# Iamctb/ImageStitching

Hardware: AMD Instinct MI355X
Metric: stitched megapixels/sec (9x12 MP vertical) (higher is better)
Workload: dtype u8

## Files before the change

imagestitching_amd/csrc/ist_ctx.h:

```cpp
#ifndef IST_CTX_H_
#define IST_CTX_H_

#include <hip/hip_runtime_api.h>

#include <memory>
#include <mutex>
#include <vector>

#include "ist_jpeg.h"

#include "ist_host.h"
#include "ist_internal.h"
#include "ist_launch.h"

struct ist_ctx {
  int device = 0;
  hipStream_t stream = nullptr;
  void* scratch_src = nullptr; size_t scratch_src_bytes = 0;
  void* scratch_dst = nullptr; size_t scratch_dst_bytes = 0;
  void* scratch_dec = nullptr; size_t scratch_dec_bytes = 0;
  void* scratch_huff = nullptr; size_t scratch_huff_bytes = 0;
  void* scratch_png = nullptr; size_t scratch_png_bytes = 0;
  void* scratch_file = nullptr; size_t scratch_file_bytes = 0;
  void* scratch_jpg = nullptr; size_t scratch_jpg_bytes = 0;
  void* scratch_arena = nullptr; size_t scratch_arena_bytes = 0;
  std::vector<hipStream_t> img_stream;
  std::vector<hipEvent_t> img_event;
  std::vector<void*> img_huff; std::vector<size_t> img_huff_bytes;
  std::unique_ptr<ist::WorkerPool> workers;
  std::vector<ist::ScanBuf> scan_bufs;
  std::vector<ist::ScanBuf> file_bufs;
  void* scratch_ent = nullptr; size_t scratch_ent_bytes = 0;
  hipStream_t render = nullptr;
  hipEvent_t render_done = nullptr;
  hipStream_t png2 = nullptr;
  hipStream_t aux = nullptr;
  static constexpr int kTablePool = 32;
  struct TableBlock { uint8_t* p; size_t bytes; };
  std::vector<TableBlock> table_pool;
  std::mutex table_mu;
  std::mutex mu;
  int png_level = 1;
  std::unique_ptr<ist::Stager> stager;
  bool timing_on = false;
  double last_ms[IST_PHASE_COUNT] = {0, 0, 0, 0, 0, 0, 0, 0};
  static constexpr int kBatchRing = 4;
  struct BatchSlot { void* host = nullptr; void* dev = nullptr; size_t bytes = 0; hipEvent_t done = nullptr; bool pending = false; };
  BatchSlot batch_ring[kBatchRing];
  int batch_next = 0;
  std::mutex batch_mu;
  struct BatchHalf {
    void* tab = nullptr; size_t tab_bytes = 0;
    void* src = nullptr; size_t src_bytes = 0;
    void* dst = nullptr; size_t dst_bytes = 0;
    void* file = nullptr; size_t file_bytes = 0;
    hipEvent_t kernel_done = nullptr;
    hipEvent_t read_done = nullptr;
  };
  BatchHalf batch_half[2];
  void* scratch_prev = nullptr; size_t scratch_prev_bytes = 0;
  hipEvent_t prev_done = nullptr; bool prev_pending = false; hipStream_t prev_last = nullptr;
  ist_job* prev_job = nullptr;
  int64_t prev_job_key[5] = {0, 0, 0, 0, 0};
  std::mutex prev_mu;
  void* prev_out = nullptr; size_t prev_out_bytes = 0;
  hipStream_t prev_stream = nullptr;
  hipEvent_t prev_ready = nullptr;
};

namespace ist {
struct DevTables {
  DevOp* ops = nullptr;
  DevCell* cells = nullptr;
  DevBand* bands = nullptr;
  int32_t* stacks = nullptr;
  DevTile* tiles = nullptr;
};
}

struct ist_job {
  ist_ctx* ctx = nullptr;
  ist::Compiled host;
  std::unique_ptr<ist::FlatTwin> flat;
  ist::DevTables flat_dt;
  uint8_t* d_tables = nullptr;
  size_t d_tables_bytes = 0;
  static constexpr int kStreams = 4;
  hipStream_t launched_on[kStreams] = {nullptr, nullptr, nullptr, nullptr};
  int n_launched_on = 0;
  bool launched = false, launched_many = false;
  std::mutex launch_mu;
  ist::DevTables dt;
  int max_image = -1;
};

#define IST_HIP(expr) do { const hipError_t e_ = (expr); if (e_ != hipSuccess) return ist::fail(IST_E_HIP, std::string(#expr) + ": " + hipGetErrorString(e_)); } while (0)
#define IST_HIP_OR(expr, msg) do { if ((expr) != hipSuccess) { (void)hipGetLastError(); return ist::fail(IST_E_HIP, msg); } } while (0)

namespace ist {

struct DeviceGuard {
  int prev = -1;
  bool ok = false;
  explicit DeviceGuard(int dev) {
    if (hipGetDevice(&prev) != hipSuccess) prev = -1;
    ok = hipSetDevice(dev) == hipSuccess;
  }
  ~DeviceGuard() { if (prev >= 0) (void)hipSetDevice(prev); }
};

int grow_device(void** p, size_t* have, size_t need);
inline size_t arena_take(size_t* off, size_t bytes) { const size_t at = *off; *off += round256(bytes); return at; }

ist_job* job_compile(ist_ctx* ctx, int64_t canvas_w, int64_t canvas_h, const uint8_t clear_rgba[4], const ist_op* ops, int n_ops,
                     const ist_image_desc* images, int n_images, int filter, const ist_region* clip);
struct TableLayout { size_t bytes[2][5] = {}; size_t at[2][5] = {}; const void* from[2][5] = {}; size_t total = 0; };
TableLayout table_layout(const ist_job& job);
void pack_tables(const TableLayout& L, uint8_t* blob);
void point_tables(ist_job* job, const TableLayout& L, uint8_t* base);
int job_launch_args(const ist_job* job, const void* const* src, const size_t* src_pitch, int n_images, void* dst, size_t dst_pitch,
                    LaunchArgs* out, const Compiled** out_run, bool* out_flat);
void note_launch_stream(ist_job* job, void* stream);
void count_flat_launches(int64_t n);

int batch_take_slot(ist_ctx* ctx, size_t bytes, ist_ctx::BatchSlot** out);

inline Stager& stager_of(ist_ctx* ctx) { if (!ctx->stager) ctx->stager.reset(new Stager(ctx->device)); return *ctx->stager; }
inline WorkerPool& workers_of(ist_ctx* ctx) { if (!ctx->workers) ctx->workers.reset(new WorkerPool()); return *ctx->workers; }
int ensure_aux(ist_ctx* ctx);
int ensure_render(ist_ctx* ctx);
int read_back_pooled(const void* dev, size_t bytes, hipStream_t stream, uint8_t** out);
int png_to_host(ist_ctx* ctx, const void* canvas, size_t pitch, int64_t w, int64_t h, void* dfile, uint8_t** out_png, int64_t* out_len,
                const std::function<int(int64_t, void*)>& need_rows = nullptr, int64_t slab_rows_hint = 0, ist_preview* preview = nullptr);

int jpeg_to_host(ist_ctx* ctx, const void* canvas, size_t pitch, int64_t w, int64_t h, int quality, int subsampling, uint8_t** out_jpeg,
                 int64_t* out_len);
int jpeg_check_options(const char* who, int quality, int subsampling);
int jpeg_check_export(const char* who, int64_t w, int64_t h, int quality, int subsampling);

int preview_check(ist_preview* pv);
inline void preview_clear(ist_preview* pv) { if (pv) { pv->width = pv->height = 0; pv->pixels = nullptr; } }
int preview_enqueue(ist_ctx* ctx, const void* src, size_t src_pitch, int64_t w, int64_t h, bool opaque, void* dst, size_t dst_pitch,
                    int32_t pw, int32_t ph, hipStream_t stream);
int preview_event(ist_ctx* ctx);
void bitmap_view(const ist_bitmap* b, int* device, const uint8_t** row0, size_t* pitch, ist_image_desc* desc);
struct PreviewTail {
  ist_ctx* ctx; const void* canvas; size_t pitch; int64_t w, h; ist_preview* pv;
  int32_t pw = 0, ph = 0;
  uint8_t* host = nullptr;
  bool queued = false;
  PreviewTail(ist_ctx* c, const void* cv, size_t p, int64_t w_, int64_t h_, ist_preview* v) : ctx(c), canvas(cv), pitch(p), w(w_), h(h_), pv(v) {}
  ~PreviewTail();
  int prepare();
  int queue(hipStream_t reader);
  int finish();
};

}

#endif
```

imagestitching_amd/csrc/ist_host.cpp:

```cpp
#include "ist_host.h"

#include <algorithm>
#include <atomic>
#include <cstring>
#include <mutex>
#include <string>
#include <thread>

#include "ist_internal.h"

namespace ist {

namespace {

constexpr size_t kPoolGranule = 2u << 20;
constexpr size_t kPoolKeepBytes = 2ull << 30;
constexpr size_t kPoolKeepBlocks = 6;

constexpr size_t kPoolKeepBatchBytes = 8ull << 30;
constexpr size_t kPoolKeepBatchBlocks = 256;

struct Block { void* p; size_t cap; bool busy; uint64_t stamp; bool batch = false; };
std::mutex g_pool_mu;
std::vector<Block>& pool() { static std::vector<Block>* v = new std::vector<Block>(); return *v; }
uint64_t g_pool_clock = 0;

void pool_enforce_class_locked(bool batch) {
  const size_t keep_bytes = batch ? kPoolKeepBatchBytes : kPoolKeepBytes, keep_blocks = batch ? kPoolKeepBatchBlocks : kPoolKeepBlocks;
  for (;;) {
    size_t idle_bytes = 0, idle = 0, oldest = SIZE_MAX;
    std::vector<Block>& v = pool();
    for (size_t i = 0; i < v.size(); ++i) {
      if (v[i].busy || v[i].batch != batch) continue;
      idle_bytes += v[i].cap; ++idle;
      if (oldest == SIZE_MAX || v[i].stamp < v[oldest].stamp) oldest = i;
    }
    if (oldest == SIZE_MAX || (idle_bytes <= keep_bytes && idle <= keep_blocks)) return;
    (void)hipHostFree(v[oldest].p);
    v.erase(v.begin() + static_cast<std::ptrdiff_t>(oldest));
  }
}

void* pool_take_class(size_t bytes, bool batch) {
  const size_t need = ((bytes ? bytes : 1) + kPoolGranule - 1) / kPoolGranule * kPoolGranule;
  {
    std::lock_guard<std::mutex> lock(g_pool_mu);
    std::vector<Block>& v = pool();
    size_t best = SIZE_MAX;
    for (size_t i = 0; i < v.size(); ++i)
      if (!v[i].busy && v[i].batch == batch && v[i].cap >= need && v[i].cap <= 2 * need && (best == SIZE_MAX || v[i].cap < v[best].cap)) best = i;
    if (best != SIZE_MAX) { v[best].busy = true; v[best].stamp = ++g_pool_clock; return v[best].p; }
  }
  void* p = nullptr;
  if (hipHostMalloc(&p, need, hipHostMallocPortable) != hipSuccess) {
    (void)hipGetLastError();
    pool_trim();
    if (hipHostMalloc(&p, need, hipHostMallocPortable) != hipSuccess) { (void)hipGetLastError(); return nullptr; }
  }
  std::lock_guard<std::mutex> lock(g_pool_mu);
  pool().push_back(Block{p, need, true, ++g_pool_clock, batch});
  return p;
}
// ... 53 lines not shown
  uint8_t* d = static_cast<uint8_t*>(it.host_dst) + p.row0 * it.host_pitch + p.col0;
  if (it.host_pitch == p.n_cols) { std::memcpy(d, chunk, p.n_rows * p.n_cols); return; }
  for (size_t r = 0; r < p.n_rows; ++r) std::memcpy(d + r * it.host_pitch, chunk + r * p.n_cols, p.n_cols);
}
inline uint8_t* dev_of(const RowsCopy& it, const Piece& p) { return static_cast<uint8_t*>(it.dev) + p.row0 * it.row + p.col0; }

}

void Stager::release_lane(Lane& l) {
  if (l.stream) (void)hipStreamSynchronize(l.stream);
  for (int s = 0; s < 2; ++s) { if (l.done[s]) (void)hipEventDestroy(l.done[s]); if (l.chunk[s]) (void)hipHostFree(l.chunk[s]); l.done[s] = nullptr; l.chunk[s] = nullptr; }
  if (l.tail) (void)hipEventDestroy(l.tail);
  if (l.stream) (void)hipStreamDestroy(l.stream);
  l.tail = nullptr; l.stream = nullptr;
}

Stager::~Stager() {
  int prev = -1;
  (void)hipGetDevice(&prev);
  if (hipSetDevice(device_) != hipSuccess) return;
  if (big_.stream) (void)hipStreamSynchronize(big_.stream);
  for (int s = 0; s < 2; ++s) { if (big_.done[s]) (void)hipEventDestroy(big_.done[s]); if (big_.piece[s]) (void)hipHostFree(big_.piece[s]); }
  if (big_.tail) (void)hipEventDestroy(big_.tail);
  if (big_.stream) (void)hipStreamDestroy(big_.stream);
  for (Lane& l : lanes_) release_lane(l);
  if (gate_) (void)hipEventDestroy(gate_);
  if (prev >= 0) (void)hipSetDevice(prev);
}

int Stager::ensure() {
  if (!lanes_.empty()) return IST_OK;
  std::vector<Lane> lanes(kLanes);
  hipEvent_t gate = nullptr;
  bool ok = hipEventCreateWithFlags(&gate, hipEventDisableTiming) == hipSuccess;
  for (Lane& l : lanes) {
    ok = ok && hipStreamCreateWithFlags(&l.stream, hipStreamNonBlocking) == hipSuccess &&
         hipEventCreateWithFlags(&l.tail, hipEventDisableTiming) == hipSuccess;
    for (int s = 0; s < 2 && ok; ++s)
      ok = hipHostMalloc(&l.chunk[s], kChunk, hipHostMallocDefault) == hipSuccess &&
           hipEventCreateWithFlags(&l.done[s], hipEventDisableTiming) == hipSuccess &&
           hipEventRecord(l.done[s], l.stream) == hipSuccess;
  }
  if (!ok) {
    (void)hipGetLastError();
    for (Lane& l : lanes) release_lane(l);
    if (gate) (void)hipEventDestroy(gate);
    return fail(IST_E_HIP, "allocating the pinned staging ring failed");
  }
  lanes_.swap(lanes);
  gate_ = gate;
  return IST_OK;
}

namespace { constexpr size_t kBigPiece = 32u << 20; constexpr int kBigPackers = 4; }

int Stager::ensure_big() {
  if (big_.stream) return IST_OK;
  Big b;
  bool ok = hipStreamCreateWithFlags(&b.stream, hipStreamNonBlocking) == hipSuccess && hipEventCreateWithFlags(&b.tail, hipEventDisableTiming) == hipSuccess;
  for (int s = 0; s < 2 && ok; ++s)
    ok = hipHostMalloc(&b.piece[s], kBigPiece, hipHostMallocDefault) == hipSuccess && hipEventCreateWithFlags(&b.done[s], hipEventDisableTiming) == hipSuccess &&
         hipEventRecord(b.done[s], b.stream) == hipSuccess;
  if (!ok) {
    (void)hipGetLastError();
    for (int s = 0; s < 2; ++s) { if (b.done[s]) (void)hipEventDestroy(b.done[s]); if (b.piece[s]) (void)hipHostFree(b.piece[s]); }
    if (b.tail) (void)hipEventDestroy(b.tail);
    if (b.stream) (void)hipStreamDestroy(b.stream);
    return fail(IST_E_HIP, "allocating the large staging pieces failed");
  }
  big_ = b;
  return IST_OK;
}

int Stager::upload_big(const std::vector<RowsCopy>& items, hipStream_t after, WorkerPool* pool) {
  if (!pool) return upload(items, after);
  std::vector<RowsCopy> small;
  bool any = false;
  for (const RowsCopy& it : items) { if (it.row == 0 || it.rows == 0) continue; if (it.row > kBigPiece) small.push_back(it); else any = true; }
  if (!small.empty()) { const int rc = upload(small, after); if (rc) return rc; }
  if (!any) return IST_OK;
  int rc = ensure_big();
  if (rc) return rc;
  for (const RowsCopy& it : items) {
    if (it.row == 0 || it.rows == 0 || it.row > kBigPiece) continue;
    if (it.host_pitch == it.row) {
      hipPointerAttribute_t attr;
      std::memset(&attr, 0, sizeof(attr));
      if (hipPointerGetAttributes(&attr, it.host_src) == hipSuccess && attr.type == hipMemoryTypeHost) {
        if (hipMemcpyAsync(it.dev, it.host_src, it.rows * it.row, hipMemcpyHostToDevice, big_.stream) != hipSuccess) { (void)hipGetLastError(); return fail(IST_E_HIP, "host-to-device copy failed"); }
        continue;
      }
      (void)hipGetLastError();
    }
    const size_t per = std::max<size_t>(1, kBigPiece / it.row);
    for (size_t r0 = 0; r0 < it.rows; r0 += per) {
      const size_t nr = std::min(per, it.rows - r0);
      const int s = static_cast<int>(big_.k++ & 1u);
      if (hipEventSynchronize(big_.done[s]) != hipSuccess) { (void)hipGetLastError(); return fail(IST_E_HIP, "host-to-device staging failed"); }
      uint8_t* piece = static_cast<uint8_t*>(big_.piece[s]);
      const int workers = static_cast<int>(std::min<size_t>(kBigPackers, std::max<size_t>(1, nr * it.row >> 20)));
      const size_t share = (nr + static_cast<size_t>(workers) - 1) / static_cast<size_t>(workers);
      auto part = [&](int w) {
        const size_t a = static_cast<size_t>(w) * share, b = std::min(nr, a + share);
        if (a >= b) return;
        const uint8_t* src = static_cast<const uint8_t*>(it.host_src) + (r0 + a) * it.host_pitch;
        if (it.host_pitch == it.row) std::memcpy(piece + a * it.row, src, (b - a) * it.row);
        else for (size_t r = a; r < b; ++r) std::memcpy(piece + r * it.row, src + (r - a) * it.host_pitch, it.row);
      };
      if (workers > 1) { pool->run(workers, part); pool->wait(); } else part(0);
      if (hipMemcpyAsync(static_cast<uint8_t*>(it.dev) + r0 * it.row, piece, nr * it.row, hipMemcpyHostToDevice, big_.stream) != hipSuccess ||
          hipEventRecord(big_.done[s], big_.stream) != hipSuccess) { (void)hipGetLastError(); return fail(IST_E_HIP, "host-to-device staging failed"); }
    }
  }
  if (hipEventRecord(big_.tail, big_.stream) != hipSuccess || hipStreamWaitEvent(after, big_.tail, 0) != hipSuccess) { (void)hipGetLastError(); return fail(IST_E_HIP, "ordering the uploads before the launch failed"); }
  return IST_OK;
}

int Stager::sync() {
  bool ok = true;
  if (big_.stream) ok = hipStreamSynchronize(big_.stream) == hipSuccess;
  for (Lane& l : lanes_) if (l.stream) ok = (hipStreamSynchronize(l.stream) == hipSuccess) && ok;
  return ok ? IST_OK : fail(IST_E_HIP, "hipStreamSynchronize failed");
}

int Stager::upload(const std::vector<RowsCopy>& items, hipStream_t after) { return run(items, true, after); }
int Stager::download(const std::vector<RowsCopy>& items, hipStream_t before) { return run(items, false, before); }

int Stager::run(const std::vector<RowsCopy>& items, bool up, hipStream_t other) {
  std::vector<Piece> pieces;
  split(items, &pieces);
  if (pieces.empty()) return IST_OK;
  int rc = ensure();
  if (rc) return rc;
  size_t total = 0;
  for (const Piece& p : pieces) total += piece_bytes(p);
  const int n_lanes = total < (2u << 20) ? 1 : static_cast<int>(std::min<size_t>(kLanes, pieces.size()));
  if (!up) {
    if (hipEventRecord(gate_, other) != hipSuccess) return fail(IST_E_HIP, "hipEventRecord failed");
    for (int l = 0; l < n_lanes; ++l)
      if (hipStreamWaitEvent(lanes_[static_cast<size_t>(l)].stream, gate_, 0) != hipSuccess) return fail(IST_E_HIP, "hipStreamWaitEvent failed");
  }
  std::atomic<size_t> next{0};
  std::atomic<int> err{0};
  auto work = [&](int li) {
    if (hipSetDevice(device_) != hipSuccess) { err = 1; return; }
    Lane& L = lanes_[static_cast<size_t>(li)];
    const Piece* pending[2] = {nullptr, nullptr};
    unsigned k = 0;
    for (;;) {
      const size_t i = next.fetch_add(1);
      if (i >= pieces.size() || err.load()) break;
      const Piece& p = pieces[i];
      const RowsCopy& it = items[p.item];
      const int s = static_cast<int>(k++ & 1u);
      if (hipEventSynchronize(L.done[s]) != hipSuccess) { err = 1; break; }
      uint8_t* chunk = static_cast<uint8_t*>(L.chunk[s]);
      if (up) {
        pack(it, p, chunk);
        if (hipMemcpyAsync(dev_of(it, p), chunk, piece_bytes(p), hipMemcpyHostToDevice, L.stream) != hipSuccess) { err = 1; break; }
      } else {
        if (pending[s]) { unpack(items[pending[s]->item], *pending[s], chunk); pending[s] = nullptr; }
        if (hipMemcpyAsync(chunk, dev_of(it, p), piece_bytes(p), hipMemcpyDeviceToHost, L.stream) != hipSuccess) { err = 1; break; }
        pending[s] = &p;
      }
      if (hipEventRecord(L.done[s], L.stream) != hipSuccess) { err = 1; break; }
// ... 69 lines not shown
```

imagestitching_amd/csrc/ist_host_stitch.cpp:

```cpp
#include <algorithm>
#include <atomic>
#include <chrono>
#include <cstdio>
#include <cstdlib>
#include <mutex>
#include <vector>

#include "ist_ctx.h"

using namespace ist;

namespace {

std::atomic<int64_t> g_duplex_stitches{0};

int render_to_scratch(ist_ctx* ctx, int64_t canvas_w, int64_t canvas_h, const uint8_t clear_rgba[4],
                      const ist_op* ops, int n_ops, const ist_image_desc* images, const uint8_t* const* src,
                      const size_t* src_pitch, int n_images, int filter, const ist_region* region,
                      int64_t* out_w, int64_t* out_h) {
  const JobPtr job(ist_job_create(ctx, canvas_w, canvas_h, clear_rgba, ops, n_ops, images, n_images, filter, region));
  if (!job) return g_last_code ? g_last_code : IST_E_INVALID;

  SourceLayout lay;
  int rc = lay.add(images, n_images, src, src_pitch, whole_bitmaps(job->host));
  if (rc) return rc;
  rc = grow_device(&ctx->scratch_src, &ctx->scratch_src_bytes, lay.bytes());
  if (rc) return rc;
  const int64_t rw = job->host.rx1 - job->host.rx0, rh = job->host.ry1 - job->host.ry0;
  const size_t pitch = static_cast<size_t>(rw) * 4;
  rc = grow_device(&ctx->scratch_dst, &ctx->scratch_dst_bytes, pitch * static_cast<size_t>(rh));
  if (rc) return rc;
  const SourceLayout::Placed at = lay.place(ctx->scratch_src);
  std::vector<RowsCopy> up;
  lay.copy_all(&up);
  rc = stager_of(ctx).upload(up, ctx->stream);
  if (rc) return rc;
  const uintptr_t biased = reinterpret_cast<uintptr_t>(ctx->scratch_dst) - (static_cast<uintptr_t>(job->host.ry0) * pitch + static_cast<uintptr_t>(job->host.rx0) * 4);
  rc = ist_job_launch(job.get(), at.ptr.data(), at.pitch.data(), n_images, reinterpret_cast<void*>(biased), pitch, ctx->stream);
  if (rc) return rc;
  IST_HIP(hipStreamSynchronize(ctx->stream));
  if (out_w) *out_w = rw;
  if (out_h) *out_h = rh;
  return IST_OK;
}

struct RowBands {
  ist_ctx* ctx = nullptr;
  bool ok = false;
  int nb = 0, n_images = 0;
  int64_t cw = 0, ch = 0;
  size_t row = 0, total = 0;
  const ist_image_desc* images = nullptr;
  std::vector<int32_t> cuts;
  std::vector<std::map<int, RowSpan>> need;
  std::vector<JobPtr> jobs;
  SourceLayout lay;
  SourceLayout::Placed at;
  std::vector<int64_t> lo, hi;
  std::vector<RowsCopy> items;
  uint8_t* canvas = nullptr;
  int64_t y0(int b) const { return cuts[static_cast<size_t>(b)]; }
  int64_t y1(int b) const { return cuts[static_cast<size_t>(b) + 1]; }

  int prepare(ist_ctx* c, int64_t canvas_w, int64_t canvas_h, const uint8_t clear[4], const ist_op* ops, int n_ops, const ist_image_desc* imgs,
              const uint8_t* const* s, const size_t* sp, int n, int filter) {
    static const bool off = tuning_mode() && std::getenv("IST_HOST_DUPLEX") && std::atoi(std::getenv("IST_HOST_DUPLEX")) == 0;
    ctx = c; cw = canvas_w; ch = canvas_h; images = imgs; n_images = n;
    row = static_cast<size_t>(cw) * 4; total = row * static_cast<size_t>(ch);
    if (off || total < (32u << 20) || n_images < 1) return IST_OK;
    nb = static_cast<int>(std::min<size_t>(16, std::max<size_t>(2, total / (40u << 20))));
    cuts.assign(static_cast<size_t>(nb) + 1, 0);
    std::vector<ist_part> parts(static_cast<size_t>(std::max(1, n_ops)) * static_cast<size_t>(nb) + 8);
    int n_parts = 0;
    {
      KeepLastError keep;
      if (ist_shard_row_cuts(ch, nb, cuts.data()) != IST_OK ||
          ist_shard_parts(ops, n_ops, cw, ch, images, n_images, filter, nb, IST_SPLIT_ROWS, parts.data(), static_cast<int>(parts.size()), &n_parts) != IST_OK)
        return IST_OK;
    }
    parts.resize(static_cast<size_t>(n_parts));
    jobs.resize(static_cast<size_t>(nb)); need.resize(static_cast<size_t>(nb));
    for (int b = 0; b < nb; ++b) {
      need[static_cast<size_t>(b)] = shard_holdings(parts_of_slot(parts, b));
      if (y0(b) >= y1(b)) continue;
      const ist_region clip{0, static_cast<int32_t>(y0(b)), static_cast<int32_t>(cw), static_cast<int32_t>(y1(b) - y0(b))};
      jobs[static_cast<size_t>(b)].reset(ist_job_create(ctx, cw, ch, clear, ops, n_ops, images, n_images, filter, &clip));
      if (!jobs[static_cast<size_t>(b)]) return g_last_code ? g_last_code : IST_E_INVALID;
    }
    std::map<int, RowSpan> whole;
    for (const auto& band : need) for (const auto& kv : band) whole[kv.first] = RowSpan{0, bitmap_h(images[kv.first])};
    int rc = lay.add(images, n_images, s, sp, whole);
    if (rc) return rc;
    rc = grow_device(&ctx->scratch_src, &ctx->scratch_src_bytes, lay.bytes());
    if (rc) return rc;
    rc = grow_device(&ctx->scratch_dst, &ctx->scratch_dst_bytes, total);
    if (rc) return rc;
    at = lay.place(ctx->scratch_src);
    lo.assign(static_cast<size_t>(n_images), -1); hi.assign(static_cast<size_t>(n_images), -1);
    canvas = static_cast<uint8_t*>(ctx->scratch_dst);
    ok = true;
    return IST_OK;
  }

  int submit(int b, hipStream_t R) {
    items.clear();
    auto send = [&](int i, int64_t r0, int64_t r1) { if (r1 > r0) items.push_back(lay.copy(i, r0, r1)); };
    for (const auto& kv : need[static_cast<size_t>(b)]) {
      const int i = kv.first;
      const int64_t a = std::max<int64_t>(0, kv.second.y0), e = std::min<int64_t>(bitmap_h(images[i]), kv.second.y1);
      if (e <= a) continue;
      int64_t& L0 = lo[static_cast<size_t>(i)]; int64_t& H0 = hi[static_cast<size_t>(i)];
      if (L0 < 0) { send(i, a, e); L0 = a; H0 = e; }
      else {
        if (a < L0) { send(i, a, L0); L0 = a; }
        if (e > H0) { send(i, H0, e); H0 = e; }
      }
    }
    if (!items.empty()) { const int rc = stager_of(ctx).upload_big(items, R, &workers_of(ctx)); if (rc) return rc; }
    return ist_job_launch(jobs[static_cast<size_t>(b)].get(), at.ptr.data(), at.pitch.data(), n_images, canvas, row, R);
  }
};

int stitch_banded_duplex(ist_ctx* ctx, const ist_plan* plan, const ist_op* ops, int n_ops, const ist_image_desc* images,
                         const uint8_t* const* src, const size_t* src_pitch, int n_images, int filter, uint8_t** out_pixels, bool* done) {
  *done = false;
  static const bool print = std::getenv("IST_TIMING") != nullptr;
  const auto t_start = std::chrono::steady_clock::now();
  auto lap = [&](const char* what) { if (print) std::fprintf(stderr, "[ist timing] host stitch: %-34s at %7.2f ms\n", what, std::chrono::duration<double, std::milli>(std::chrono::steady_clock::now() - t_start).count()); };
  RowBands rb;
  int rc = rb.prepare(ctx, plan->canvas_w, plan->canvas_h, kTransparent, ops, n_ops, images, src, src_pitch, n_images, filter);
  if (rc) return rc;
  if (!rb.ok) return IST_OK;
  rc = ensure_aux(ctx);
  if (rc) return rc;
  lap("band jobs compiled, scratch");
  uint8_t* host = static_cast<uint8_t*>(pool_take(rb.total));
  if (!host) return fail(IST_E_NOMEM, "out of pinned host memory for the result");
  std::vector<hipEvent_t> ev(static_cast<size_t>(rb.nb), nullptr);
  hipStream_t R = ctx->stream, D = ctx->aux;
  auto finish = [&](int code) {
    (void)hipStreamSynchronize(R); (void)hipStreamSynchronize(D); (void)stager_of(ctx).sync();
    for (hipEvent_t e : ev) if (e) (void)hipEventDestroy(e);
    if (code != IST_OK) pool_give(host);
    return code;
  };
  bool first = true;
  for (int b = 0; b < rb.nb; ++b) {
    const int64_t y0 = rb.y0(b), y1 = rb.y1(b);
    if (y0 >= y1) continue;
    rc = rb.submit(b, R);
    if (rc) return finish(rc);
    hipEvent_t& e = ev[static_cast<size_t>(b)];
    if (hipEventCreateWithFlags(&e, hipEventDisableTiming) != hipSuccess || hipEventRecord(e, R) != hipSuccess || hipStreamWaitEvent(D, e, 0) != hipSuccess ||
        hipMemcpyAsync(host + static_cast<size_t>(y0) * rb.row, rb.canvas + static_cast<size_t>(y0) * rb.row, static_cast<size_t>(y1 - y0) * rb.row, hipMemcpyDeviceToHost, D) != hipSuccess) {
      (void)hipGetLastError();
      return finish(fail(IST_E_HIP, "queueing a band's readback failed"));
    }
    if (first) { lap("first band queued"); first = false; }
  }
  lap("last band queued");
  if (hipStreamSynchronize(D) != hipSuccess || hipStreamSynchronize(R) != hipSuccess) { (void)hipGetLastError(); return finish(fail(IST_E_HIP, "result readback failed")); }
  lap("last band in host memory");
  g_duplex_stitches.fetch_add(1, std::memory_order_relaxed);
  *out_pixels = host;
  *done = true;
  return finish(IST_OK);
}

int render_png_banded(ist_ctx* ctx, int64_t canvas_w, int64_t canvas_h, const uint8_t clear_rgba[4], const ist_op* ops, int n_ops,
                      const ist_image_desc* images, const uint8_t* const* src, const size_t* src_pitch, int n_images, int filter,
                      uint8_t** out_png, int64_t* out_len, ist_preview* preview) {
  RowBands rb;
  int rc = rb.prepare(ctx, canvas_w, canvas_h, clear_rgba ? clear_rgba : kTransparent, ops, n_ops, images, src, src_pitch, n_images, filter);
  if (rc) return rc;
  if (!rb.ok) return 1;
  rc = ensure_render(ctx);
  if (rc) return rc;
  hipStream_t R = ctx->render;
  std::vector<hipEvent_t> ev(static_cast<size_t>(rb.nb), nullptr);
  int next = 0;
  auto need_rows = [&](int64_t y_end, void* reader_) -> int {
    hipStream_t reader = static_cast<hipStream_t>(reader_);
    int last = -1;
    for (int b = 0; b < rb.nb; ++b) {
      if (rb.y0(b) >= rb.y1(b)) continue;
      if (rb.y0(b) >= y_end) break;
      if (b >= next) {
        const int rc2 = rb.submit(b, R);
        if (rc2) return rc2;
        if (hipEventCreateWithFlags(&ev[static_cast<size_t>(b)], hipEventDisableTiming) != hipSuccess || hipEventRecord(ev[static_cast<size_t>(b)], R) != hipSuccess) {
          (void)hipGetLastError(); return fail(IST_E_HIP, "hipEventRecord failed");
        }
        next = b + 1;
      }
      last = b;
    }
    if (last >= 0 && hipStreamWaitEvent(reader, ev[static_cast<size_t>(last)], 0) != hipSuccess) { (void)hipGetLastError(); return fail(IST_E_HIP, "ordering the export behind the render failed"); }
    return IST_OK;
  };
  int64_t hint = 0;
  for (int b = 0; b < rb.nb; ++b) hint = std::max<int64_t>(hint, rb.y1(b) - rb.y0(b));
  rc = png_to_host(ctx, rb.canvas, rb.row, canvas_w, canvas_h, nullptr, out_png, out_len, need_rows, hint, preview);
  (void)hipStreamSynchronize(R); (void)stager_of(ctx).sync(); (void)hipStreamSynchronize(ctx->stream);
  for (hipEvent_t e : ev) if (e) (void)hipEventDestroy(e);
  if (rc == IST_OK) g_duplex_stitches.fetch_add(1, std::memory_order_relaxed);
  return rc;
}

int render_png(ist_ctx* ctx, int64_t canvas_w, int64_t canvas_h, const uint8_t clear_rgba[4], const ist_op* ops, int n_ops,
               const ist_image_desc* images, const uint8_t* const* src, const size_t* src_pitch, int n_images, int filter,
               uint8_t** out_png, int64_t* out_len, ist_preview* preview) {
  *out_png = nullptr; *out_len = 0;
  std::lock_guard<std::mutex> lock(ctx->mu);
  DeviceGuard g(ctx->device);
  int rc = render_png_banded(ctx, canvas_w, canvas_h, clear_rgba, ops, n_ops, images, src, src_pitch, n_images, filter, out_png, out_len, preview);
  if (rc != 1) return rc;
  rc = render_to_scratch(ctx, canvas_w, canvas_h, clear_rgba, ops, n_ops, images, src, src_pitch, n_images, filter, nullptr, nullptr, nullptr);
  if (rc) return rc;
  return png_to_host(ctx, ctx->scratch_dst, static_cast<size_t>(canvas_w) * 4, canvas_w, canvas_h, nullptr, out_png, out_len, nullptr, 0, preview);
}

}

extern "C" {

int64_t ist_debug_duplex_stitches(void) { return g_duplex_stitches.load(); }

int ist_render_rgba8(ist_ctx* ctx, int64_t canvas_w, int64_t canvas_h, const uint8_t clear_rgba[4],
                     const ist_op* ops, int n_ops, const ist_image_desc* images, const uint8_t* const* src,
                     const size_t* src_pitch, int n_images, int filter, const ist_region* region, uint8_t* dst,
                     size_t dst_pitch) {
  if (!ctx) return fail(IST_E_NO_CONTEXT, "无法获取绘图上下文");
  if (!dst) return fail(IST_E_INVALID, "ist_render_rgba8: dst is NULL");
  std::lock_guard<std::mutex> lock(ctx->mu);
  DeviceGuard g(ctx->device);
  int64_t rw = canvas_w, rh = canvas_h;
  if (region) {
    const int64_t rx = std::max<int64_t>(0, region->x), ry = std::max<int64_t>(0, region->y);
    rw = std::min<int64_t>(canvas_w, static_cast<int64_t>(region->x) + region->w) - rx;
    rh = std::min<int64_t>(canvas_h, static_cast<int64_t>(region->y) + region->h) - ry;
  }
  if (rw > 0 && dst_pitch < static_cast<size_t>(rw) * 4) return fail(IST_E_INVALID, "dst_pitch too small");
  int rc = render_to_scratch(ctx, canvas_w, canvas_h, clear_rgba, ops, n_ops, images, src, src_pitch, n_images, filter, region, &rw, &rh);
  if (rc) return rc;
  std::vector<RowsCopy> down{RowsCopy{ctx->scratch_dst, nullptr, dst, dst_pitch, static_cast<size_t>(rw) * 4, static_cast<size_t>(rh)}};
  return stager_of(ctx).download(down, ctx->stream);
}

int ist_render_png(ist_ctx* ctx, int64_t canvas_w, int64_t canvas_h, const uint8_t clear_rgba[4], const ist_op* ops,
                   int n_ops, const ist_image_desc* images, const uint8_t* const* src, const size_t* src_pitch,
                   int n_images, int filter, uint8_t** out_png, int64_t* out_len) {
  if (!ctx) return fail(IST_E_NO_CONTEXT, "无法获取绘图上下文");
  if (!out_png || !out_len) return fail(IST_E_INVALID, "ist_render_png: NULL output");
  return render_png(ctx, canvas_w, canvas_h, clear_rgba, ops, n_ops, images, src, src_pitch, n_images, filter, out_png, out_len, nullptr);
}

int ist_stitch_png_preview(ist_ctx* ctx, const ist_image_desc* images, const uint8_t* const* src, const size_t* src_pitch,
// ... 91 lines not shown
```

imagestitching_amd/csrc/ist_runtime.cpp:

```cpp
#include <hip/hip_runtime_api.h>

#include <algorithm>
#include <atomic>
#include <cstdlib>
#include <cstring>
#include <functional>
#include <memory>
#include <mutex>

#include "ist_ctx.h"

using namespace ist;

namespace ist {
int ctx_png_level(const ist_ctx* ctx) { return ctx ? ctx->png_level : 0; }
int ctx_png_scratch(ist_ctx* ctx, size_t need, void** p) {
  const int rc = grow_device(&ctx->scratch_png, &ctx->scratch_png_bytes, need);
  *p = ctx->scratch_png;
  return rc;
}

static std::atomic<int64_t> g_dev_allocs{0};
int dev_malloc(void** p, size_t bytes) {
  g_dev_allocs.fetch_add(1, std::memory_order_relaxed);
  return static_cast<int>(hipMalloc(p, bytes));
}
void dev_free(void* p) { if (p) (void)hipFree(p); }

int grow_device(void** p, size_t* have, size_t need) {
  if (*have >= need) return IST_OK;
  if (*p) { dev_free(*p); *p = nullptr; *have = 0; }
  if (dev_malloc(p, need) != 0) { (void)hipGetLastError(); return fail(IST_E_NOMEM, "out of device memory (" + std::to_string(need >> 20) + " MiB)"); }
  *have = need;
  return IST_OK;
}

int read_back_pooled(const void* dev, size_t bytes, hipStream_t stream, uint8_t** out) {
  uint8_t* host = static_cast<uint8_t*>(pool_take(bytes));
  if (!host) return fail(IST_E_NOMEM, "out of pinned host memory for the result");
  if (hipMemcpyAsync(host, dev, bytes, hipMemcpyDeviceToHost, stream) != hipSuccess || hipStreamSynchronize(stream) != hipSuccess) {
    (void)hipGetLastError();
    pool_give(host);
    return fail(IST_E_HIP, "result readback failed");
  }
  *out = host;
  return IST_OK;
}

static int ensure_stream(hipStream_t* s, bool lowest = false) {
  if (*s) return IST_OK;
  int lo = 0, hi = 0;
  (void)hipDeviceGetStreamPriorityRange(&lo, &hi);
  if (hipStreamCreateWithPriority(s, hipStreamNonBlocking, lowest ? lo : hi) != hipSuccess) { (void)hipGetLastError(); *s = nullptr; return fail(IST_E_HIP, "hipStreamCreate failed"); }
  return IST_OK;
}
int ensure_aux(ist_ctx* ctx) {
  static const bool lowest = tuning_mode() && std::getenv("IST_AUX_PRIORITY") && !std::atoi(std::getenv("IST_AUX_PRIORITY"));
  return ensure_stream(&ctx->aux, lowest);
}
int ensure_render(ist_ctx* ctx) { return ensure_stream(&ctx->render); }

int png_to_host(ist_ctx* ctx, const void* canvas, size_t pitch, int64_t w, int64_t h, void* dfile, uint8_t** out_png, int64_t* out_len,
                const std::function<int(int64_t, void*)>& need_rows_in, int64_t slab_rows_hint, ist_preview* preview) {
  PreviewTail tail(ctx, canvas, pitch, w, h, preview);
  std::function<int(int64_t, void*)> with_preview;
  if (preview) {
    const int rc = tail.prepare();
    if (rc) return rc;
    with_preview = [&](int64_t y_end, void* reader) -> int {
      const int rc2 = need_rows_in ? need_rows_in(y_end, reader) : IST_OK;
      if (rc2 || y_end < h) return rc2;
      return tail.queue(static_cast<hipStream_t>(reader));
    };
  }
  const std::function<int(int64_t, void*)>& need_rows = preview ? with_preview : need_rows_in;
  const int64_t cap = ist_png_bound(w, h);
  if (!dfile) {
    const int rc = grow_device(&ctx->scratch_file, &ctx->scratch_file_bytes, static_cast<size_t>(cap));
    if (rc) return rc;
    dfile = ctx->scratch_file;
  }
  int64_t len = 0;
  if (ctx->png_level > 0) {
    { const int rc = ensure_aux(ctx); if (rc) return rc; }
    uint8_t* host = static_cast<uint8_t*>(pool_take(static_cast<size_t>(cap)));
    if (!host) return fail(IST_E_NOMEM, "out of pinned host memory for the result");
    if (!ctx->png2 && hipStreamCreateWithFlags(&ctx->png2, hipStreamNonBlocking) != hipSuccess) { (void)hipGetLastError(); ctx->png2 = nullptr; }
    const int rc = png_encode_device_deflate(ctx, canvas, pitch, w, h, dfile, cap, &len, ctx->stream, host, ctx->aux, need_rows, slab_rows_hint, ctx->png2);
    if (rc) { (void)hipStreamSynchronize(ctx->aux); (void)hipStreamSynchronize(ctx->stream); if (ctx->png2) (void)hipStreamSynchronize(ctx->png2); pool_give(host); return rc; }
    if (preview) { const int rc2 = tail.finish(); if (rc2) { pool_give(host); return rc2; } }
    *out_png = host; *out_len = len;
    return IST_OK;
  }
  int rc = need_rows ? need_rows(h, ctx->stream) : IST_OK;
  if (rc) return rc;
  rc = ist_png_encode_device(ctx, canvas, pitch, w, h, dfile, cap, &len, ctx->stream);
  if (rc) return rc;
  uint8_t* host = nullptr;
  rc = read_back_pooled(dfile, static_cast<size_t>(len), ctx->stream, &host);
  if (rc) return rc;
  if (preview) { rc = tail.finish(); if (rc) { pool_give(host); return rc; } }
  *out_png = host; *out_len = len;
  return IST_OK;
}

}

extern "C" {

int64_t ist_debug_device_allocs(void) { return g_dev_allocs.load(std::memory_order_relaxed); }

int ist_device_count(void) {
  int n = 0;
// ... 8 lines not shown
  DeviceGuard g(device);
  if (!g.ok) { fail(IST_E_NO_DEVICE, "hipSetDevice failed"); return nullptr; }
  std::unique_ptr<ist_ctx> c(new ist_ctx);
  c->device = device;
  if (hipStreamCreateWithFlags(&c->stream, hipStreamNonBlocking) != hipSuccess) {
    fail(IST_E_HIP, "hipStreamCreate failed");
    return nullptr;
  }
  return c.release();
}

int ist_ctx_set_png_level(ist_ctx* ctx, int level) {
  if (!ctx) return fail(IST_E_NO_CONTEXT, "无法获取绘图上下文");
  if (level < 0 || level > 1) return fail(IST_E_INVALID, "PNG level must be 0 (stored) or 1 (compressed)");
  ctx->png_level = level;
  return IST_OK;
}

int ist_ctx_sync(ist_ctx* ctx) {
  if (!ctx) return fail(IST_E_NO_CONTEXT, "无法获取绘图上下文");
  DeviceGuard g(ctx->device);
  bool ok = hipStreamSynchronize(ctx->stream) == hipSuccess;
  if (ctx->aux) ok = (hipStreamSynchronize(ctx->aux) == hipSuccess) && ok;
  if (ctx->render) ok = (hipStreamSynchronize(ctx->render) == hipSuccess) && ok;
  if (ctx->png2) ok = (hipStreamSynchronize(ctx->png2) == hipSuccess) && ok;
  if (ctx->prev_stream) ok = (hipStreamSynchronize(ctx->prev_stream) == hipSuccess) && ok;
  if (ctx->stager) ok = (ctx->stager->sync() == IST_OK) && ok;
  if (!ok) { (void)hipGetLastError(); return fail(IST_E_HIP, "hipStreamSynchronize failed"); }
  return IST_OK;
}

void ist_ctx_destroy(ist_ctx* ctx) {
  if (!ctx) return;
  DeviceGuard g(ctx->device);
  if (ctx->stream) (void)hipStreamSynchronize(ctx->stream);
  if (ctx->aux) (void)hipStreamSynchronize(ctx->aux);
  if (ctx->prev_job) ist_job_destroy(ctx->prev_job);
  if (ctx->prev_stream) { (void)hipStreamSynchronize(ctx->prev_stream); (void)hipStreamDestroy(ctx->prev_stream); }
  if (ctx->prev_done) { (void)hipEventSynchronize(ctx->prev_done); (void)hipEventDestroy(ctx->prev_done); }
  if (ctx->prev_ready) (void)hipEventDestroy(ctx->prev_ready);
  dev_free(ctx->scratch_prev);
  dev_free(ctx->prev_out);
  dev_free(ctx->scratch_src);
  dev_free(ctx->scratch_dst);
  dev_free(ctx->scratch_dec);
  dev_free(ctx->scratch_huff);
  dev_free(ctx->scratch_png);
  dev_free(ctx->scratch_file);
  dev_free(ctx->scratch_jpg);
  dev_free(ctx->scratch_arena);
  dev_free(ctx->scratch_ent);
  for (hipStream_t st : ctx->img_stream) if (st) { (void)hipStreamSynchronize(st); (void)hipStreamDestroy(st); }
  for (hipEvent_t ev : ctx->img_event) if (ev) (void)hipEventDestroy(ev);
  for (void* q : ctx->img_huff) dev_free(q);
  if (ctx->aux) (void)hipStreamDestroy(ctx->aux);
  if (ctx->render) { (void)hipStreamSynchronize(ctx->render); (void)hipStreamDestroy(ctx->render); }
  if (ctx->png2) { (void)hipStreamSynchronize(ctx->png2); (void)hipStreamDestroy(ctx->png2); }
  if (ctx->render_done) (void)hipEventDestroy(ctx->render_done);
  for (const ist_ctx::TableBlock& b : ctx->table_pool) dev_free(b.p);
  for (ist_ctx::BatchSlot& s : ctx->batch_ring) {
    if (s.done) { (void)hipEventSynchronize(s.done); (void)hipEventDestroy(s.done); }
    if (s.host) (void)hipHostFree(s.host);
    dev_free(s.dev);
  }
  for (ist_ctx::BatchHalf& h : ctx->batch_half) {
    dev_free(h.tab); dev_free(h.src); dev_free(h.dst); dev_free(h.file);
    if (h.kernel_done) (void)hipEventDestroy(h.kernel_done);
    if (h.read_done) (void)hipEventDestroy(h.read_done);
  }
  ctx->workers.reset();
  ctx->stager.reset();
  if (ctx->stream) (void)hipStreamDestroy(ctx->stream);
  delete ctx;
}

static std::atomic<int64_t> g_flat_launches{0};

int64_t ist_debug_flat_launches(void) { return g_flat_launches.load(); }

}

namespace ist {
void count_flat_launches(int64_t n) { g_flat_launches.fetch_add(n, std::memory_order_relaxed); }

ist_job* job_compile(ist_ctx* ctx, int64_t canvas_w, int64_t canvas_h, const uint8_t clear_rgba[4], const ist_op* ops, int n_ops,
                     const ist_image_desc* images, int n_images, int filter, const ist_region* clip) {
  if (!ctx) { fail(IST_E_NO_CONTEXT, "无法获取绘图上下文"); return nullptr; }
  if (n_images > kMaxImages) { fail(IST_E_UNSUPPORTED, "more than 128 images in one launch"); return nullptr; }
  std::unique_ptr<ist_job> job(new ist_job);
  job->ctx = ctx;
  if (compile_ops(canvas_w, canvas_h, clear_rgba ? clear_rgba : kTransparent, ops, n_ops, images, n_images, filter,
                  clip, &job->host) != IST_OK)
    return nullptr;
  for (const DevOp& o : job->host.ops) job->max_image = std::max(job->max_image, o.image);
  job->flat = compile_flat_twin(canvas_w, canvas_h, clear_rgba ? clear_rgba : kTransparent, ops, n_ops, images, n_images, filter, job->host);
  return job.release();
}

TableLayout table_layout(const ist_job& job) {
  TableLayout L;
  const Compiled* hs[2] = {&job.host, job.flat ? &job.flat->host : nullptr};
  for (int t = 0; t < 2; ++t) {
    if (!hs[t]) continue;
    const Compiled& h = *hs[t];
    const size_t b[5] = {h.ops.size() * sizeof(DevOp), h.cells.size() * sizeof(DevCell), h.bands.size() * sizeof(DevBand),
                         h.stacks.size() * sizeof(int32_t), h.tiles.size() * sizeof(DevTile)};
// ... 186 lines not shown
```

Measured before the change: 823,500.

## Overlap band job compilation with uploads and coalesce staged upload pieces

Band jobs after the first are now compiled on a background thread, and each band's launch waits only for its own job, so host-side compilation overlaps with staging and GPU work. Staged host-to-device uploads are planned across items into evenly sized pieces that may each hold several images, replacing per-item piece chunking, and they are packed byte-range-parallel. The number of packer threads now follows a CPU budget read from affinity and cgroup quotas. Per-band events are pooled in the context instead of being created and destroyed per call. This adds thread and synchronization complexity, and the band compile now runs on a separate thread that sets the device itself.

```diff
diff --git a/imagestitching_amd/csrc/ist_ctx.h b/imagestitching_amd/csrc/ist_ctx.h
--- a/imagestitching_amd/csrc/ist_ctx.h
+++ b/imagestitching_amd/csrc/ist_ctx.h
@@ -35,6 +35,7 @@
   hipEvent_t render_done = nullptr;
   hipStream_t png2 = nullptr;
   hipStream_t aux = nullptr;
+  std::vector<hipEvent_t> band_event;
   static constexpr int kTablePool = 32;
   struct TableBlock { uint8_t* p; size_t bytes; };
   std::vector<TableBlock> table_pool;
@@ -129,6 +130,7 @@
 inline WorkerPool& workers_of(ist_ctx* ctx) { if (!ctx->workers) ctx->workers.reset(new WorkerPool()); return *ctx->workers; }
 int ensure_aux(ist_ctx* ctx);
 int ensure_render(ist_ctx* ctx);
+int band_events(ist_ctx* ctx, int n);
 int read_back_pooled(const void* dev, size_t bytes, hipStream_t stream, uint8_t** out);
 int png_to_host(ist_ctx* ctx, const void* canvas, size_t pitch, int64_t w, int64_t h, void* dfile, uint8_t** out_png, int64_t* out_len,
                 const std::function<int(int64_t, void*)>& need_rows = nullptr, int64_t slab_rows_hint = 0, ist_preview* preview = nullptr);
diff --git a/imagestitching_amd/csrc/ist_host.cpp b/imagestitching_amd/csrc/ist_host.cpp
--- a/imagestitching_amd/csrc/ist_host.cpp
+++ b/imagestitching_amd/csrc/ist_host.cpp
@@ -2,12 +2,14 @@
 
 #include <algorithm>
 #include <atomic>
+#include <cstdlib>
 #include <cstring>
 #include <mutex>
 #include <string>
 #include <thread>
 
 #include "ist_internal.h"
+#include "ist_upload_plan.h"
 
 namespace ist {
 
@@ -167,7 +169,19 @@
   return IST_OK;
 }
 
-namespace { constexpr size_t kBigPiece = 32u << 20; constexpr int kBigPackers = 4; }
+namespace {
+
+constexpr size_t kBigPiece = 32u << 20;
+
+int big_packers() {
+  static const int n = []() {
+    if (tuning_mode() && std::getenv("IST_PACKERS")) return std::min(WorkerPool::kMaxThreads, std::max(1, std::atoi(std::getenv("IST_PACKERS"))));
+    return packers_for_budget(cpu_budget());
+  }();
+  return n;
+}
+
+}
 
 int Stager::ensure_big() {
   if (big_.stream) return IST_OK;
@@ -196,36 +210,45 @@
   if (!any) return IST_OK;
   int rc = ensure_big();
   if (rc) return rc;
-  for (const RowsCopy& it : items) {
+  std::vector<UploadItem> plan_items(items.size());
+  std::vector<UploadSource> from(items.size());
+  for (size_t k = 0; k < items.size(); ++k) {
+    const RowsCopy& it = items[k];
+    plan_items[k].row = it.row; plan_items[k].rows = it.rows;
+    from[k] = UploadSource{it.host_src, it.host_pitch};
     if (it.row == 0 || it.rows == 0 || it.row > kBigPiece) continue;
     if (it.host_pitch == it.row) {
       hipPointerAttribute_t attr;
       std::memset(&attr, 0, sizeof(attr));
       if (hipPointerGetAttributes(&attr, it.host_src) == hipSuccess && attr.type == hipMemoryTypeHost) {
         if (hipMemcpyAsync(it.dev, it.host_src, it.rows * it.row, hipMemcpyHostToDevice, big_.stream) != hipSuccess) { (void)hipGetLastError(); return fail(IST_E_HIP, "host-to-device copy failed"); }
+        plan_items[k].direct = true;
         continue;
       }
       (void)hipGetLastError();
     }
-    const size_t per = std::max<size_t>(1, kBigPiece / it.row);
-    for (size_t r0 = 0; r0 < it.rows; r0 += per) {
-      const size_t nr = std::min(per, it.rows - r0);
-      const int s = static_cast<int>(big_.k++ & 1u);
-      if (hipEventSynchronize(big_.done[s]) != hipSuccess) { (void)hipGetLastError(); return fail(IST_E_HIP, "host-to-device staging failed"); }
-      uint8_t* piece = static_cast<uint8_t*>(big_.piece[s]);
-      const int workers = static_cast<int>(std::min<size_t>(kBigPackers, std::max<size_t>(1, nr * it.row >> 20)));
-      const size_t share = (nr + static_cast<size_t>(workers) - 1) / static_cast<size_t>(workers);
-      auto part = [&](int w) {
-        const size_t a = static_cast<size_t>(w) * share, b = std::min(nr, a + share);
-        if (a >= b) return;
-        const uint8_t* src = static_cast<const uint8_t*>(it.host_src) + (r0 + a) * it.host_pitch;
-        if (it.host_pitch == it.row) std::memcpy(piece + a * it.row, src, (b - a) * it.row);
-        else for (size_t r = a; r < b; ++r) std::memcpy(piece + r * it.row, src + (r - a) * it.host_pitch, it.row);
-      };
-      if (workers > 1) { pool->run(workers, part); pool->wait(); } else part(0);
-      if (hipMemcpyAsync(static_cast<uint8_t*>(it.dev) + r0 * it.row, piece, nr * it.row, hipMemcpyHostToDevice, big_.stream) != hipSuccess ||
-          hipEventRecord(big_.done[s], big_.stream) != hipSuccess) { (void)hipGetLastError(); return fail(IST_E_HIP, "host-to-device staging failed"); }
-    }
+  }
+  UploadPlan plan;
+  plan_upload_pieces(plan_items.data(), plan_items.size(), kBigPiece, &plan);
+  for (const UploadPiece& pc : plan.pieces) {
+    const int s = static_cast<int>(big_.k++ & 1u);
+    if (hipEventSynchronize(big_.done[s]) != hipSuccess) { (void)hipGetLastError(); return fail(IST_E_HIP, "host-to-device staging failed"); }
+    uint8_t* piece = static_cast<uint8_t*>(big_.piece[s]);
+    const UploadSeg* segs = plan.segs.data() + pc.seg0;
+    const size_t workers = std::min<size_t>(static_cast<size_t>(big_packers()), std::max<size_t>(1, pc.bytes >> 20));
+    const size_t share = piece_share(pc.bytes, workers);
+    auto part = [&](int w) { pack_piece_bytes(plan, pc, plan_items.data(), from.data(), static_cast<size_t>(w) * share, static_cast<size_t>(w + 1) * share, piece); };
+    if (workers > 1) { pool->run(static_cast<int>(workers), part); pool->wait(); } else part(0);
+    for (size_t q = 0; q < pc.n_segs; ++q) {
+      const UploadSeg& sg = segs[q];
+      const RowsCopy& it = items[sg.item];
+      if (hipMemcpyAsync(static_cast<uint8_t*>(it.dev) + sg.row0 * it.row, piece + sg.at, sg.n_rows * it.row, hipMemcpyHostToDevice, big_.stream) != hipSuccess) {
+        (void)hipGetLastError();
+        (void)hipEventRecord(big_.done[s], big_.stream);
+        return fail(IST_E_HIP, "host-to-device staging failed");
+      }
+    }
+    if (hipEventRecord(big_.done[s], big_.stream) != hipSuccess) { (void)hipGetLastError(); return fail(IST_E_HIP, "host-to-device staging failed"); }
   }
   if (hipEventRecord(big_.tail, big_.stream) != hipSuccess || hipStreamWaitEvent(after, big_.tail, 0) != hipSuccess) { (void)hipGetLastError(); return fail(IST_E_HIP, "ordering the uploads before the launch failed"); }
   return IST_OK;
diff --git a/imagestitching_amd/csrc/ist_host_stitch.cpp b/imagestitching_amd/csrc/ist_host_stitch.cpp
--- a/imagestitching_amd/csrc/ist_host_stitch.cpp
+++ b/imagestitching_amd/csrc/ist_host_stitch.cpp
@@ -1,9 +1,12 @@
 #include <algorithm>
 #include <atomic>
 #include <chrono>
+#include <condition_variable>
 #include <cstdio>
 #include <cstdlib>
 #include <mutex>
+#include <string>
+#include <thread>
 #include <vector>
 
 #include "ist_ctx.h"
@@ -59,6 +62,13 @@
   std::vector<int64_t> lo, hi;
   std::vector<RowsCopy> items;
   uint8_t* canvas = nullptr;
+  std::thread compiler;
+  std::mutex compile_mu;
+  std::condition_variable compile_cv;
+  int n_compiled = 0, compile_rc = IST_OK;
+  std::string compile_msg;
+  std::atomic<bool> give_up{false};
+  ~RowBands() { give_up = true; if (compiler.joinable()) compiler.join(); }
   int64_t y0(int b) const { return cuts[static_cast<size_t>(b)]; }
   int64_t y1(int b) const { return cuts[static_cast<size_t>(b) + 1]; }
 
@@ -80,13 +90,15 @@
     }
     parts.resize(static_cast<size_t>(n_parts));
     jobs.resize(static_cast<size_t>(nb)); need.resize(static_cast<size_t>(nb));
-    for (int b = 0; b < nb; ++b) {
-      need[static_cast<size_t>(b)] = shard_holdings(parts_of_slot(parts, b));
-      if (y0(b) >= y1(b)) continue;
+    for (int b = 0; b < nb; ++b) need[static_cast<size_t>(b)] = shard_holdings(parts_of_slot(parts, b));
+    auto compile = [this, clear, ops, n_ops, filter](int b) -> int {
+      if (y0(b) >= y1(b)) return IST_OK;
       const ist_region clip{0, static_cast<int32_t>(y0(b)), static_cast<int32_t>(cw), static_cast<int32_t>(y1(b) - y0(b))};
       jobs[static_cast<size_t>(b)].reset(ist_job_create(ctx, cw, ch, clear, ops, n_ops, images, n_images, filter, &clip));
-      if (!jobs[static_cast<size_t>(b)]) return g_last_code ? g_last_code : IST_E_INVALID;
-    }
+      return jobs[static_cast<size_t>(b)] ? IST_OK : (g_last_code ? g_last_code : IST_E_INVALID);
+    };
+    if (const int rc0 = compile(0)) return rc0;
+    n_compiled = 1;
     std::map<int, RowSpan> whole;
     for (const auto& band : need) for (const auto& kv : band) whole[kv.first] = RowSpan{0, bitmap_h(images[kv.first])};
     int rc = lay.add(images, n_images, s, sp, whole);
@@ -98,7 +110,28 @@
     at = lay.place(ctx->scratch_src);
     lo.assign(static_cast<size_t>(n_images), -1); hi.assign(static_cast<size_t>(n_images), -1);
     canvas = static_cast<uint8_t*>(ctx->scratch_dst);
+    rc = band_events(ctx, nb);
+    if (rc) return rc;
+    if (nb > 1)
+      compiler = std::thread([this, compile]() {
+        DeviceGuard g(ctx->device);
+        for (int b = 1; b < nb && !give_up.load(); ++b) {
+          const int rc_b = g.ok ? compile(b) : fail(IST_E_NO_DEVICE, "hipSetDevice failed");
+          std::lock_guard<std::mutex> lock(compile_mu);
+          if (rc_b) { compile_rc = rc_b; compile_msg = g_last_error; n_compiled = nb; }
+          else n_compiled = b + 1;
+          compile_cv.notify_all();
+          if (rc_b) return;
+        }
+      });
     ok = true;
+    return IST_OK;
+  }
+
+  int wait_compiled(int b) {
+    std::unique_lock<std::mutex> lock(compile_mu);
+    compile_cv.wait(lock, [&]() { return n_compiled > b; });
+    if (compile_rc && !jobs[static_cast<size_t>(b)] && y0(b) < y1(b)) return fail(compile_rc, compile_msg);
     return IST_OK;
   }
 
@@ -117,6 +150,7 @@
       }
     }
     if (!items.empty()) { const int rc = stager_of(ctx).upload_big(items, R, &workers_of(ctx)); if (rc) return rc; }
+    if (const int rc = wait_compiled(b)) return rc;
     return ist_job_launch(jobs[static_cast<size_t>(b)].get(), at.ptr.data(), at.pitch.data(), n_images, canvas, row, R);
   }
 };
@@ -136,11 +170,10 @@
   lap("band jobs compiled, scratch");
   uint8_t* host = static_cast<uint8_t*>(pool_take(rb.total));
   if (!host) return fail(IST_E_NOMEM, "out of pinned host memory for the result");
-  std::vector<hipEvent_t> ev(static_cast<size_t>(rb.nb), nullptr);
+  const std::vector<hipEvent_t>& ev = ctx->band_event;
   hipStream_t R = ctx->stream, D = ctx->aux;
   auto finish = [&](int code) {
     (void)hipStreamSynchronize(R); (void)hipStreamSynchronize(D); (void)stager_of(ctx).sync();
-    for (hipEvent_t e : ev) if (e) (void)hipEventDestroy(e);
     if (code != IST_OK) pool_give(host);
     return code;
   };
@@ -150,8 +183,8 @@
     if (y0 >= y1) continue;
     rc = rb.submit(b, R);
     if (rc) return finish(rc);
-    hipEvent_t& e = ev[static_cast<size_t>(b)];
-    if (hipEventCreateWithFlags(&e, hipEventDisableTiming) != hipSuccess || hipEventRecord(e, R) != hipSuccess || hipStreamWaitEvent(D, e, 0) != hipSuccess ||
+    hipEvent_t e = ev[static_cast<size_t>(b)];
+    if (hipEventRecord(e, R) != hipSuccess || hipStreamWaitEvent(D, e, 0) != hipSuccess ||
         hipMemcpyAsync(host + static_cast<size_t>(y0) * rb.row, rb.canvas + static_cast<size_t>(y0) * rb.row, static_cast<size_t>(y1 - y0) * rb.row, hipMemcpyDeviceToHost, D) != hipSuccess) {
       (void)hipGetLastError();
       return finish(fail(IST_E_HIP, "queueing a band's readback failed"));
@@ -177,7 +210,7 @@
   rc = ensure_render(ctx);
   if (rc) return rc;
   hipStream_t R = ctx->render;
-  std::vector<hipEvent_t> ev(static_cast<size_t>(rb.nb), nullptr);
+  const std::vector<hipEvent_t>& ev = ctx->band_event;
   int next = 0;
   auto need_rows = [&](int64_t y_end, void* reader_) -> int {
     hipStream_t reader = static_cast<hipStream_t>(reader_);
@@ -188,7 +221,7 @@
       if (b >= next) {
         const int rc2 = rb.submit(b, R);
         if (rc2) return rc2;
-        if (hipEventCreateWithFlags(&ev[static_cast<size_t>(b)], hipEventDisableTiming) != hipSuccess || hipEventRecord(ev[static_cast<size_t>(b)], R) != hipSuccess) {
+        if (hipEventRecord(ev[static_cast<size_t>(b)], R) != hipSuccess) {
           (void)hipGetLastError(); return fail(IST_E_HIP, "hipEventRecord failed");
         }
         next = b + 1;
@@ -202,7 +235,6 @@
   for (int b = 0; b < rb.nb; ++b) hint = std::max<int64_t>(hint, rb.y1(b) - rb.y0(b));
   rc = png_to_host(ctx, rb.canvas, rb.row, canvas_w, canvas_h, nullptr, out_png, out_len, need_rows, hint, preview);
   (void)hipStreamSynchronize(R); (void)stager_of(ctx).sync(); (void)hipStreamSynchronize(ctx->stream);
-  for (hipEvent_t e : ev) if (e) (void)hipEventDestroy(e);
   if (rc == IST_OK) g_duplex_stitches.fetch_add(1, std::memory_order_relaxed);
   return rc;
 }
diff --git a/imagestitching_amd/csrc/ist_runtime.cpp b/imagestitching_amd/csrc/ist_runtime.cpp
--- a/imagestitching_amd/csrc/ist_runtime.cpp
+++ b/imagestitching_amd/csrc/ist_runtime.cpp
@@ -59,6 +59,14 @@
   return ensure_stream(&ctx->aux, lowest);
 }
 int ensure_render(ist_ctx* ctx) { return ensure_stream(&ctx->render); }
+int band_events(ist_ctx* ctx, int n) {
+  while (static_cast<int>(ctx->band_event.size()) < n) {
+    hipEvent_t e = nullptr;
+    if (hipEventCreateWithFlags(&e, hipEventDisableTiming) != hipSuccess) { (void)hipGetLastError(); return fail(IST_E_HIP, "hipEventCreate failed"); }
+    ctx->band_event.push_back(e);
+  }
+  return IST_OK;
+}
 
 int png_to_host(ist_ctx* ctx, const void* canvas, size_t pitch, int64_t w, int64_t h, void* dfile, uint8_t** out_png, int64_t* out_len,
                 const std::function<int(int64_t, void*)>& need_rows_in, int64_t slab_rows_hint, ist_preview* preview) {
@@ -173,6 +181,7 @@
   dev_free(ctx->scratch_ent);
   for (hipStream_t st : ctx->img_stream) if (st) { (void)hipStreamSynchronize(st); (void)hipStreamDestroy(st); }
   for (hipEvent_t ev : ctx->img_event) if (ev) (void)hipEventDestroy(ev);
+  for (hipEvent_t ev : ctx->band_event) if (ev) (void)hipEventDestroy(ev);
   for (void* q : ctx->img_huff) dev_free(q);
   if (ctx->aux) (void)hipStreamDestroy(ctx->aux);
   if (ctx->render) { (void)hipStreamSynchronize(ctx->render); (void)hipStreamDestroy(ctx->render); }
diff --git a/imagestitching_amd/csrc/ist_upload_plan.cpp b/imagestitching_amd/csrc/ist_upload_plan.cpp
--- /dev/null
+++ b/imagestitching_amd/csrc/ist_upload_plan.cpp
@@ -0,0 +1,108 @@
+#include "ist_upload_plan.h"
+
+#include <algorithm>
+#include <cstdio>
+#include <cstdlib>
+#include <cstring>
+#include <string>
+
+#ifdef __linux__
+#include <sched.h>
+#endif
+
+namespace ist {
+
+void plan_upload_pieces(const UploadItem* items, size_t n_items, size_t cap, UploadPlan* out) {
+  out->segs.clear(); out->pieces.clear(); out->total = 0; out->widest = 0;
+  auto planned = [&](const UploadItem& it) { return !it.direct && it.row != 0 && it.rows != 0 && it.row <= cap; };
+  for (size_t i = 0; i < n_items; ++i)
+    if (planned(items[i])) { out->total += items[i].row * items[i].rows; out->widest = std::max(out->widest, items[i].row); }
+  const size_t T = out->total;
+  if (!T) return;
+  const size_t n0 = (T + cap - 1) / cap;
+  size_t i = 0, r = 0, done = 0;
+  for (size_t k = 1; done < T; ++k) {
+    const size_t target = k >= n0 ? T : static_cast<size_t>(static_cast<unsigned __int128>(T) * k / n0);
+    const size_t budget = std::min(target - done, cap);
+    UploadPiece p{out->segs.size(), 0, 0};
+    while (i < n_items) {
+      const UploadItem& it = items[i];
+      if (!planned(it) || r == it.rows) { ++i; r = 0; continue; }
+      const size_t take = std::min((budget - p.bytes) / it.row, it.rows - r);
+      if (!take) break;
+      out->segs.push_back(UploadSeg{static_cast<uint32_t>(i), r, take, p.bytes});
+      p.bytes += take * it.row; r += take; ++p.n_segs;
+    }
+    if (p.n_segs) { out->pieces.push_back(p); done += p.bytes; }
+  }
+}
+
+void pack_piece_bytes(const UploadPlan& plan, const UploadPiece& pc, const UploadItem* items, const UploadSource* src, size_t a, size_t b, uint8_t* piece) {
+  b = std::min(b, pc.bytes);
+  for (size_t q = 0; q < pc.n_segs && a < b; ++q) {
+    const UploadSeg& sg = plan.segs[pc.seg0 + q];
+    const size_t row = items[sg.item].row, pitch = src[sg.item].pitch;
+    size_t lo = std::max(a, sg.at);
+    const size_t hi = std::min(b, sg.at + sg.n_rows * row);
+    if (lo >= hi) continue;
+    const uint8_t* from = static_cast<const uint8_t*>(src[sg.item].host) + sg.row0 * pitch;
+    if (pitch == row) { std::memcpy(piece + lo, from + (lo - sg.at), hi - lo); continue; }
+    while (lo < hi) {
+      const size_t off = lo - sg.at, r = off / row, c = off % row, n = std::min(row - c, hi - lo);
+      std::memcpy(piece + lo, from + r * pitch + c, n);
+      lo += n;
+    }
+  }
+}
+
+namespace {
+
+#ifdef __linux__
+int quota_of(const std::string& path) {
+  std::FILE* f = std::fopen(path.c_str(), "r");
+  if (!f) return 0;
+  char q[32] = {0};
+  long long period = 0;
+  const int got = std::fscanf(f, "%31s %lld", q, &period);
+  std::fclose(f);
+  if (got != 2 || period <= 0 || !std::strcmp(q, "max")) return 0;
+  const long long quota = std::atoll(q);
+  if (quota <= 0) return 0;
+  return static_cast<int>(std::min<long long>((quota + period - 1) / period, 1 << 20));
+}
+#endif
+
+int compute_budget() {
+  int n = 0;
+#ifdef __linux__
+  cpu_set_t set;
+  CPU_ZERO(&set);
+  if (sched_getaffinity(0, sizeof(set), &set) == 0) n = CPU_COUNT(&set);
+  std::string group = "/";
+  if (std::FILE* f = std::fopen("/proc/self/cgroup", "r")) {
+    char line[4096];
+    while (std::fgets(line, sizeof(line), f))
+      if (!std::strncmp(line, "0::", 3)) { group = line + 3; while (!group.empty() && (group.back() == '\n' || group.back() == '/')) group.pop_back(); }
+    std::fclose(f);
+  }
+  for (;;) {
+    const int q = quota_of("/sys/fs/cgroup" + group + "/cpu.max");
+    if (q > 0 && (n <= 0 || q < n)) n = q;
+    const size_t slash = group.rfind('/');
+    if (group.empty() || slash == std::string::npos) break;
+    group.resize(slash);
+  }
+#endif
+  return std::max(1, n);
+}
+
+}
+
+int cpu_budget() {
+  static const int budget = compute_budget();
+  return budget;
+}
+
+int packers_for_budget(int budget) { return std::min(4, std::max(2, budget / 2)); }
+
+}
diff --git a/imagestitching_amd/csrc/ist_upload_plan.h b/imagestitching_amd/csrc/ist_upload_plan.h
--- /dev/null
+++ b/imagestitching_amd/csrc/ist_upload_plan.h
@@ -0,0 +1,34 @@
+#ifndef IST_UPLOAD_PLAN_H_
+#define IST_UPLOAD_PLAN_H_
+
+#include <cstddef>
+#include <cstdint>
+#include <vector>
+
+namespace ist {
+
+struct UploadItem {
+  size_t row = 0, rows = 0;
+  bool direct = false;
+};
+struct UploadSeg { uint32_t item; size_t row0, n_rows; size_t at; };
+struct UploadPiece { size_t seg0, n_segs, bytes; };
+struct UploadPlan {
+  std::vector<UploadSeg> segs;
+  std::vector<UploadPiece> pieces;
+  size_t total = 0;
+  size_t widest = 0;
+};
+
+void plan_upload_pieces(const UploadItem* items, size_t n_items, size_t cap, UploadPlan* out);
+
+inline size_t piece_share(size_t bytes, size_t workers) { return ((bytes + workers - 1) / workers + 63) & ~static_cast<size_t>(63); }
+struct UploadSource { const void* host; size_t pitch; };
+void pack_piece_bytes(const UploadPlan& plan, const UploadPiece& pc, const UploadItem* items, const UploadSource* src, size_t a, size_t b, uint8_t* piece);
+
+int cpu_budget();
+int packers_for_budget(int budget);
+
+}
+
+#endif
```

Measured after the change: 813,600. 0.988x the previous value.
